# smileyenot983/reconstructor

Hardware: AMD Instinct MI355X
Metric: descriptor pair-distances/s + BA LM-iterations/s (1k cams, 100k pts) (higher is better)
Workload: dtype f16+f64

## Files before the change

reconstructor_amd/csrc/ctx.hip:

```cpp
#include "rcn_internal.h"

#include <cstdlib>

extern "C" {

const char *rcn_version(void)
{
#ifdef RCN_DIAG
    return "reconstructor_amd 0.19 (gfx950) DIAGNOSTIC BUILD";
#else
    return "reconstructor_amd 0.19 (gfx950)";
#endif
}

int rcn_create(int device_id, rcn_ctx **out)
{
    if (!out) return RCN_ERR_ARG;
    *out = nullptr;
    int n = 0;
    if (hipGetDeviceCount(&n) != hipSuccess || n <= 0 || device_id < 0 || device_id >= n)
        return RCN_ERR_NO_DEVICE;
    rcn_ctx *ctx = new rcn_ctx();
    ctx->device = device_id;
    if (hipSetDevice(device_id) != hipSuccess ||
        hipGetDeviceProperties(&ctx->prop, device_id) != hipSuccess) {
        delete ctx;
        return RCN_ERR_NO_DEVICE;
    }
    if (std::string(ctx->prop.gcnArchName).rfind("gfx950", 0) != 0) {
        delete ctx;
        return RCN_ERR_NO_DEVICE;
    }
    if (hipStreamCreateWithFlags(&ctx->own_stream, hipStreamNonBlocking) != hipSuccess) {
        delete ctx;
        return RCN_ERR_HIP;
    }
    ctx->stream = ctx->own_stream;
    if (int rcc = rcn_chol_create(ctx)) { delete ctx; return rcc; }
    if (hipEventCreateWithFlags(&ctx->ba_pair_ev, hipEventDisableTiming) != hipSuccess) { delete ctx; return RCN_ERR_HIP; }
    for (auto &e : ctx->ba_tev)
        if (hipEventCreate(&e) != hipSuccess) { delete ctx; return RCN_ERR_HIP; }
    ctx->ba_ev_made = true;
    if (hipHostMalloc(reinterpret_cast<void **>(&ctx->ba_host_scal), 16 * sizeof(double), hipHostMallocDefault) != hipSuccess) { (void)hipGetLastError(); ctx->ba_host_scal = nullptr; }
    else memset(ctx->ba_host_scal, 0, 16 * sizeof(double));
#ifdef RCN_DIAG
    const char *w4 = std::getenv("RCN_COARSE_W4");
    ctx->coarse_w4 = w4 && w4[0] == '1';
    const char *s16 = std::getenv("RCN_COARSE_S16");
    ctx->coarse_shape = s16 ? (s16[0] == '1' ? 1 : 0) : -1;
    const char *i8 = std::getenv("RCN_COARSE_I8");
    ctx->coarse_i8_off = i8 && i8[0] == '0';
    const char *i8s = std::getenv("RCN_COARSE_I8_S16");
    ctx->coarse_i8_shape = i8s ? (i8s[0] == '1' ? 1 : 0) : -1;
    const char *fe = std::getenv("RCN_FORCE_EXACT");
    ctx->force_exact = fe && fe[0] == '1';
    const char *mi8 = std::getenv("RCN_MID_I8");
    ctx->mid_i8_off = mi8 && mi8[0] == '0';
    const char *rrp = std::getenv("RCN_RERANK_PASS");
    ctx->rerank_pass = rrp && rrp[0] == '1';
    const char *flp = std::getenv("RCN_FILTER_PASS");
    ctx->filter_pass = flp && flp[0] == '1';
    const char *nio = getenv("RCN_MATCH_NO_ORDER");
    ctx->no_item_order = nio && nio[0] == '1';
    const char *ab = std::getenv("RCN_COARSE_ABL");
    ctx->ablate = ab ? std::atoi(ab) : 0;
    const char *bat = std::getenv("RCN_BA_SCHUR_ATOMICS");
    ctx->ba_atomics = bat && bat[0] == '1';
    const char *bps = getenv("RCN_PAIR_SMALL");
    if (bps) ctx->ba_pair_small = bps[0] != '0';
    const char *btf = getenv("RCN_BA_TRSV_FWD");
    ctx->ba_trsv_fwd = btf && btf[0] == '1';
    if (const char *bm = std::getenv("RCN_BA_MIRROR")) if (bm[0] == '0' && ctx->ba_host_scal) { (void)hipHostFree(ctx->ba_host_scal); ctx->ba_host_scal = nullptr; }
    const char *ch = std::getenv("RCN_CHUNK_ROWS");
    if (ch && std::atoll(ch) > 0) ctx->chunk_rows = std::atoll(ch);
    const char *mr = std::getenv("RCN_MID_ROWS");
    if (mr && std::atoll(mr) >= 0) ctx->mid_rows = std::max<long long>(1, std::atoll(mr));
#endif
    memset(&ctx->last_stats, 0, sizeof(ctx->last_stats));
    *out = ctx;
    return RCN_OK;
}

void rcn_destroy(rcn_ctx *ctx)
{
    if (!ctx) return;
    (void)hipSetDevice(ctx->device);
    (void)hipStreamSynchronize(ctx->stream);
    rcn_match_release(ctx);
    rcn_int_ham_release(ctx);
    rcn_int_guided_release(ctx);
    rcn_int_tracks_release(ctx);
    rcn_int_mvs_release(ctx);
    DevBuf *bufs[] = {&ctx->img_table, &ctx->pairs_dev, &ctx->groups_dev, &ctx->cand, &ctx->owner,
                      &ctx->fb_list, &ctx->sv_list, &ctx->counters, &ctx->out_tmp, &ctx->cnt_tmp, &ctx->scale_dev, &ctx->desc_bad, &ctx->kp_ws, &ctx->sg_ws, &ctx->sg_scores, &ctx->gnn_ws, &ctx->gnn_mdesc, &ctx->sp_ws, &ctx->sp_out, &ctx->sift_ws, &ctx->sift_pyr, &ctx->retr_ws, &ctx->retr_out, &ctx->img_ws, &ctx->orb_ws, &ctx->orb_pyr, &ctx->orb_tab};
    for (DevBuf *b : bufs) b->release();
    for (DevBuf &b : ctx->ba_ws) b.release();
    ctx->ba_loss_ws.release();
    ctx->lm_ws.release();
    ctx->tri_ws.release();
    ctx->tri_dws.release();
    ctx->fm_ws.release();
    ctx->fm_state.release();
    ctx->fm_csr.release(); ctx->fm_pairs.release();
    for (auto &kv : ctx->coords) kv.second.first.release();
    ctx->corr.release();
    ctx->corr_ws.release(); ctx->corr_hws.release(); ctx->corr_slots.release(); ctx->att_ws.release();
    if (ctx->corr_ev) (void)hipEventDestroy(ctx->corr_ev);
    ctx->lid.release(); ctx->lid_slot_off.release(); ctx->lid_hws.release(); ctx->nvt_ws.release();
    if (ctx->nvt_ev) (void)hipEventDestroy(ctx->nvt_ev);
    if (ctx->img_ev) (void)hipEventDestroy(ctx->img_ev);
// ... 50 lines not shown
```

reconstructor_amd/csrc/match.hip:

```cpp
#include "rcn_internal.h"

#include <algorithm>
#include <cmath>

typedef _Float16 half8 __attribute__((ext_vector_type(8)));
typedef float f32x16 __attribute__((ext_vector_type(16)));
typedef float f32x4 __attribute__((ext_vector_type(4)));
typedef unsigned u32x4 __attribute__((ext_vector_type(4)));

#define RCN_TBL_BYTES ((RCN_GROUP * 24 + 127) / 128 * 128)
#define RCN_NBUF 4
#define RCN_PD 2
#define RCN_CHUNK_ROWS (1ll << 27)
#define RCN_BT 64
#define RCN_PAD_HN 1.0e30f
#define RCN_I8_IDX_MASK ((1u << RCN_I8_IDX_BITS) - 1u)
#define RCN_I8_PAD_ACC ((1 << (32 - RCN_I8_IDX_BITS)) - 1)
#define RCN_I8_BT 128
#ifndef RCN_I8_EARLY_OPEN
#define RCN_I8_EARLY_OPEN 1
#endif
#define RCN_I8_RES_MAX 8.01
#define RCN_I8_M_MAX 720.0
#define RCN_I8_PEAK_MAX 8.0
// ... 1529 lines not shown
        const unsigned cnt = a.ccount[r];
        if (cnt > (unsigned)RCN_MIDCAP) {
            if (lane == 0) a.fb2_list[atomicAdd(a.fb2_count, 1u)] = e;
            continue;
        }
        const ImgDev qi = a.imgs[a.pairs[2 * pair]];
        const ImgDev ti = a.imgs[a.pairs[2 * pair + 1]];
        double b0 = INFINITY, b1 = INFINITY;
        int i0 = 0x7FFFFFFF, i1 = 0x7FFFFFFF;
        if (lane < (int)cnt) {
            i0 = a.clist[(size_t)r * RCN_MIDCAP + lane];
            b0 = exact_d2<true>(qi.f32 + (size_t)q * a.D, ti.f32 + (size_t)i0 * a.D, a.D);
            if (!(b0 < INFINITY)) { b0 = INFINITY; i0 = 0x7FFFFFFF; }
        }
        for (int o = 32; o; o >>= 1) {
            const double c0 = __shfl_xor(b0, o), c1 = __shfl_xor(b1, o);
            const int j0 = __shfl_xor(i0, o), j1 = __shfl_xor(i1, o);
            merge_top2(b0, i0, b1, i1, c0, j0, c1, j1);
        }
        if (lane == 0) a.out[(size_t)pair * a.out_stride + q] = ratio_pass(b0, b1, a.ratio) ? i0 : -1;
    }
}

__global__ void k_unique_claim(const ImgDev *__restrict__ imgs, const int32_t *__restrict__ pairs,
                               const int32_t *__restrict__ out, int64_t out_stride,
                               int32_t *__restrict__ owner, int owner_stride, int qblocks, int pair_base)
{
    const int pl = blockIdx.x / qblocks, pair = pair_base + pl;
    const int q = (blockIdx.x - pl * qblocks) * blockDim.x + threadIdx.x;
    if (q >= imgs[pairs[2 * pair]].K) return;
    const int t = out[(size_t)pair * out_stride + q];
    if (t >= 0) atomicMin(owner + (size_t)pair * owner_stride + t, q);
}

__global__ void k_unique_emit(const ImgDev *__restrict__ imgs, const int32_t *__restrict__ pairs,
                              int32_t *__restrict__ out, int64_t out_stride,
                              const int32_t *__restrict__ owner, int owner_stride,
                              int32_t *__restrict__ counts, int qblocks, int pair_base)
{
    const int pl = blockIdx.x / qblocks, pair = pair_base + pl;
    const int q = (blockIdx.x - pl * qblocks) * blockDim.x + threadIdx.x;
    if (q >= out_stride) return;
    int32_t *o = out + (size_t)pair * out_stride + q;
    bool keep = false;
    if (q < imgs[pairs[2 * pair]].K) {
        const int t = *o;
        keep = t >= 0 && owner[(size_t)pair * owner_stride + t] == q;
    }
    if (!keep) *o = -1;
    const unsigned long long m = __ballot(keep);
    if ((threadIdx.x & 63) == 0 && m) atomicAdd(counts + pair, (int)__popcll(m));
}

__global__ __launch_bounds__(256) void k_unique_pair(const ImgDev *__restrict__ imgs, const int32_t *__restrict__ pairs,
                                                     int32_t *__restrict__ out, int64_t out_stride,
                                                     int32_t *__restrict__ counts, int pair_base)
{
    __shared__ int owner[RCN_UNIQ_LDS];
    __shared__ int wsum[4];
    const int pair = pair_base + blockIdx.x, t = threadIdx.x;
    const int Kq = imgs[pairs[2 * pair]].K, Kt = imgs[pairs[2 * pair + 1]].K;
    for (int i = t; i < Kt; i += 256) owner[i] = 0x7fffffff;
    __syncthreads();
    int32_t *row = out + (size_t)pair * out_stride;
    for (int q = t; q < Kq; q += 256) {
        const int tr = row[q];
        if (tr >= 0) atomicMin(&owner[tr], q);
    }
    __syncthreads();
    int kept = 0;
    for (int q0 = 0; q0 < out_stride; q0 += 256) {
        const int q = q0 + t;
        bool keep = false;
        if (q < out_stride) {
            const int tr = q < Kq ? row[q] : -1;
            keep = tr >= 0 && owner[tr] == q;
            if (!keep && (q >= Kq || tr >= 0)) row[q] = -1;
        }
        kept += (int)__popcll(__ballot(keep));
    }
    if ((t & 63) == 0) wsum[t >> 6] = kept;
    __syncthreads();
    if (t == 0) counts[pair] = wsum[0] + wsum[1] + wsum[2] + wsum[3];
}

__global__ void k_stats_acc(unsigned *c, int mid, unsigned midrows)
{
    if (threadIdx.x != 0 || blockIdx.x != 0) return;
    c[4] += c[0];
    c[5] += c[1];
    c[6] += mid ? c[2] + (c[0] > midrows ? c[0] - midrows : 0u) : c[0];
}

static int pad_dim(int D)
{
    if (D <= 32) return 32;
    if (D <= 64) return 64;
    if (D <= 128) return 128;
    if (D <= 256) return 256;
    return 0;
}

template <typename Kernel>
static int resident_grid(rcn_ctx *ctx, Kernel kernel, int &per_cu)
{
    if (per_cu <= 0) {
        int nb = 0;
        if (hipOccupancyMaxActiveBlocksPerMultiprocessor(&nb, kernel, 64, 0) != hipSuccess || nb < 1) nb = 4;
        per_cu = nb;
    }
    return ctx->prop.multiProcessorCount * per_cu;
}
static int rerank_grid(rcn_ctx *ctx) { static int per_cu = 0; return resident_grid(ctx, k_rerank_lds, per_cu); }
static void launch_mid_exact(rcn_ctx *ctx, const MidArgs &ma, hipStream_t st)
{
    static int per_cu = 0;
    if (ma.D <= XG_ROWF) k_mid_exact<<<resident_grid(ctx, k_mid_exact, per_cu), 64, 0, st>>>(ma);
    else k_mid_exact_wide<<<ctx->prop.multiProcessorCount * 4, 256, 0, st>>>(ma);
}

static hipError_t launch_rowstats(rcn_ctx *ctx, const float *x, int rows, int D, double *nrm2, unsigned *cnt)
{
    ctx->hist_rows += rows;
    unsigned long long *mx = reinterpret_cast<unsigned long long *>(cnt + 2);
    if (D % 4 == 0 && (reinterpret_cast<uintptr_t>(x) & 15) == 0)
        k_rowstats<true><<<std::max(1, std::min((rows + 15) / 16, 4096)), 256, 0, ctx->stream>>>(x, rows, D, nrm2, cnt, mx, cnt + RCN_HIST_WORD);
    else
        k_rowstats<false><<<std::max(1, std::min((rows + 3) / 4, 4096)), 256, 0, ctx->stream>>>(x, rows, D, nrm2, cnt, mx, cnt + RCN_HIST_WORD);
    return hipGetLastError();
}

static void free_image(ImgHost &im)
{
// ... 551 lines not shown
                e = launch_coarse<128>(ctx, ca, blocks); break;
            default: e = launch_coarse<256>(ctx, ca, blocks); break;
            }
        }
    }
    RCN_HIP(e);
    if (ctx->i8_allowed) {
#ifdef RCN_DIAG
        if (ctx->coarse_i8_shape == 0) e = launch_coarse_i8<0, 0>(ctx, ca, blocks);
        else if (ctx->ablate == 1) e = launch_coarse_i8<1, 1>(ctx, ca, blocks);
        else if (ctx->ablate == 16) e = launch_coarse_i8<16, 1>(ctx, ca, blocks);
        else if (ctx->ablate == 32) e = launch_coarse_i8<32, 1>(ctx, ca, blocks);
        else
#endif
        e = launch_coarse_i8<0, 1>(ctx, ca, blocks);
        RCN_HIP(e);
    }
    return RCN_OK;
}

struct MidSource {
    const uint2 *cand;
    const unsigned long long *fb_list;
    const unsigned *fb_count;
    const float *thr_in;
    const unsigned *tacc_in;
    uint32_t midrows;
};

static int launch_mid_tier(rcn_ctx *ctx, const grid::GridPlan &pl, const RerankArgs &ra, unsigned *ccnt, const MidSource &src, bool defer_rows)
{
    const grid::MidLayout &mo = pl.mid_ws;
    const int n_slots = ctx->grid_shape.n_slots, cus = ctx->prop.multiProcessorCount;
    hipStream_t st = ctx->stream;
    char *mw = ctx->mid_ws.as<char>();
    MidArgs ma;
    memset(&ma, 0, sizeof(ma));
    ma.imgs = ra.imgs; ma.pairs = ra.pairs; ma.cand = src.cand; ma.fb_list = src.fb_list; ma.fb_count = src.fb_count;
    ma.thr_in = src.thr_in; ma.tacc_in = src.tacc_in;
    ma.sorted = (unsigned long long *)(mw + mo.sorted); ma.thr = (float *)(mw + mo.thr); ma.ccount = (unsigned *)(mw + mo.cc); ma.tacc = (unsigned *)(mw + mo.tacc);
    ma.clist = (int32_t *)(mw + mo.cl); ma.fb2_list = (unsigned long long *)(mw + mo.fb2);
    ma.hist = (unsigned *)(mw + mo.bins); ma.offs = ma.hist + (n_slots + 1); ma.cursor = ma.offs + (n_slots + 1); ma.ibase = ma.cursor + (n_slots + 1);
    ma.n_items = ccnt + 3; ma.fb2_count = ccnt + 2;
    ma.out = ra.out; ma.out_stride = ra.out_stride; ma.sc = ra.sc; ma.n_slots = n_slots; ma.kq_stride = pl.kq_stride; ma.D = ra.D;
    ma.all_to_fallback = ra.all_to_fallback; ma.idx_mask = pl.idx_mask; ma.ratio = ra.ratio; ma.midrows = src.midrows;
    if (defer_rows) {
        k_mid_defer<<<cus * 2, 256, 0, st>>>(ma, (unsigned long long *)(mw + mo.def), (float *)(mw + mo.defthr), (unsigned *)(mw + mo.deftacc), ccnt, (unsigned)mo.rows_cap);
        k_mid_defer_commit<<<1, 64, 0, st>>>(ccnt, (unsigned)mo.rows_cap);
    }
    k_mid_hist<<<cus * 4, 256, 0, st>>>(ma);
    k_mid_bins<<<1, 1024, 0, st>>>(ma);
    k_mid_scatter<<<cus * 4, 256, 0, st>>>(ma);
    k_mid_eval<<<cus * 4, 256, 0, st>>>(ma);
    if (pl.mid_i8) k_mid_eval_i8<<<dim3((unsigned)n_slots * MI8_TILES, (unsigned)pl.mid_i8_grid_y), 256, 0, st>>>(ma);
    launch_mid_exact(ctx, ma, st);
    RCN_HIP(hipGetLastError());
    k_exact_rows_lds<<<cus * 8, 64 * EX_WAVES, 0, st>>>(ra.imgs, ra.pairs, ma.fb2_list, ma.fb2_count, ra.D, ra.ratio, ra.out, ra.out_stride);
    RCN_HIP(hipGetLastError());
    return RCN_OK;
}

static int launch_unique(rcn_ctx *ctx, const grid::GridPlan &pl, const RerankArgs &ra, int32_t *counts_dev, int p0, int np)
{
    hipStream_t st = ctx->stream;
    if (pl.uniq_lds) {
        if (!pl.defer) k_unique_pair<<<np, 256, 0, st>>>(ra.imgs, ra.pairs, ra.out, ra.out_stride, counts_dev, p0);
    } else {
        const int qblocks = (pl.kq_max + 255) / 256, eblocks = (int)((ra.out_stride + 255) / 256);
        if (pl.kq_max > 0) k_unique_claim<<<dim3((unsigned)qblocks * (unsigned)np), 256, 0, st>>>(ra.imgs, ra.pairs, ra.out, ra.out_stride, ctx->owner.as<int32_t>(), pl.owner_stride, qblocks, p0);
        RCN_HIP(hipGetLastError());
        k_unique_emit<<<dim3((unsigned)eblocks * (unsigned)np), 256, 0, st>>>(ra.imgs, ra.pairs, ra.out, ra.out_stride, ctx->owner.as<int32_t>(), pl.owner_stride, counts_dev, eblocks, p0);
    }
    RCN_HIP(hipGetLastError());
    return RCN_OK;
}

int rcn_int_match_grid(rcn_ctx *ctx, const int32_t *pairs_host, int32_t n_pairs, float ratio,
                           int32_t *out_dev, int64_t out_stride, int32_t *counts_dev)
{
    if (!pairs_host && n_pairs > 0) {
        std::vector<int32_t> ids;
        for (const auto &kv : ctx->images)
            if (kv.first != INT32_MIN && kv.first != INT32_MIN + 1) ids.push_back(kv.first);
        const int64_t want = (int64_t)ids.size() * ((int64_t)ids.size() - 1) / 2;
        if (want != n_pairs) { ctx->set_error("rcn_match_grid: pairs == NULL needs n_pairs = n (n - 1) / 2 over the resident images"); return RCN_ERR_ARG; }
        std::vector<int32_t> &all = ctx->all_pairs_host;
        all.clear();
        for (size_t i = 0; i < ids.size(); ++i)
            for (size_t j = i + 1; j < ids.size(); ++j) { all.push_back(ids[i]); all.push_back(ids[j]); }
        pairs_host = all.data();
    }
    if (n_pairs < 0 || (n_pairs > 0 && (!pairs_host || !out_dev || !counts_dev))) {
        ctx->set_error("rcn_match_grid: bad argument");
        return RCN_ERR_ARG;
    }
    memset(&ctx->last_stats, 0, sizeof(ctx->last_stats));
    if (n_pairs == 0) return RCN_OK;
    RCN_HIP(hipSetDevice(ctx->device));
    int rc = rcn_int_prepare_all(ctx);
    if (rc) return rc;

    if ((rc = fill_grid_shape(ctx, pairs_host, n_pairs))) return rc;
    const grid::GridShape &gs = ctx->grid_shape;
    grid::GridPlan &pl = ctx->grid;
    grid::plan_grid(gs, pl);
    if (out_stride < pl.kq_max) {
        ctx->set_error("rcn_match_grid: out_stride smaller than a query image's K");
// ... 365 lines not shown
{
    if (!ctx || !model) return RCN_ERR_ARG;
    std::lock_guard<std::mutex> lk(ctx->mu);
    if (!ctx->scale_dev.p || !ctx->prepared) { ctx->set_error("rcn_diag_i8: nothing prepared"); return RCN_ERR_ARG; }
    RCN_HIP(hipSetDevice(ctx->device));
    ScaleDev m;
    RCN_HIP(hipMemcpyAsync(&m, ctx->scale_dev.p, sizeof(ScaleDev), hipMemcpyDeviceToHost, ctx->stream));
    RCN_HIP(hipStreamSynchronize(ctx->stream));
    model[0] = m.coarse_i8; model[1] = m.s; model[2] = m.bias; model[3] = m.rho; model[4] = m.tau; model[5] = m.n_max;
    model[6] = ctx->i8_allowed ? 1.0 : 0.0; model[7] = 0.0;
    if (!q_host && !hn_host && !norms_host) return RCN_OK;
    auto it = ctx->images.find(img_id);
    if (it == ctx->images.end()) { ctx->set_error("rcn_diag_i8: image id not resident"); return RCN_ERR_NOT_FOUND; }
    if (!m.coarse_i8 || !it->second.i8n) { ctx->set_error("rcn_diag_i8: the resident set holds no int8 copies"); return RCN_ERR_UNSUPPORTED; }
    const ImgHost &im = it->second;
    if (im.K <= 0) return RCN_OK;
    std::vector<int8_t> raw((size_t)im.K * 256);
    std::vector<float> nn((size_t)im.K * 2);
    RCN_HIP(hipMemcpyAsync(raw.data(), im.f16, raw.size(), hipMemcpyDeviceToHost, ctx->stream));
    if (hn_host) RCN_HIP(hipMemcpyAsync(hn_host, im.hn, (size_t)im.K * sizeof(int32_t), hipMemcpyDeviceToHost, ctx->stream));
    RCN_HIP(hipMemcpyAsync(nn.data(), im.i8n, nn.size() * sizeof(float), hipMemcpyDeviceToHost, ctx->stream));
    RCN_HIP(hipStreamSynchronize(ctx->stream));
    if (q_host)
        for (int r = 0; r < im.K; ++r)
            for (int c = 0; c < 16; ++c) memcpy(q_host + (size_t)r * 256 + 16 * c, raw.data() + (size_t)r * 256 + ((c ^ (r & 15)) << 4), 16);
    if (norms_host) memcpy(norms_host, nn.data(), nn.size() * sizeof(float));
    return RCN_OK;
}
#endif

#ifdef RCN_DIAG
int rcn_diag_mid(rcn_ctx *ctx, int64_t *n_rows, unsigned long long *sorted_host, uint32_t *tacc_host, uint32_t *ccount_host, int32_t *clist_host, int64_t cap)
{
    if (!ctx || !n_rows) return RCN_ERR_ARG;
    std::lock_guard<std::mutex> lk(ctx->mu);
    if (!ctx->grid.mid || !ctx->mid_ws.p || ctx->last_chunks != 1) { ctx->set_error("rcn_diag_mid: the last grid call left no single pass of the middle tier"); return RCN_ERR_UNSUPPORTED; }
    RCN_HIP(hipSetDevice(ctx->device));
    const grid::MidLayout &mo = ctx->grid.mid_ws;
    unsigned c0 = 0;
    RCN_HIP(hipMemcpyAsync(&c0, ctx->counters.as<unsigned>() + 8, sizeof(unsigned), hipMemcpyDeviceToHost, ctx->stream));
    RCN_HIP(hipStreamSynchronize(ctx->stream));
    const size_t n = std::min<size_t>(c0, mo.rows_cap);
    *n_rows = (int64_t)n;
    if (n == 0 || (!sorted_host && !tacc_host && !ccount_host && !clist_host)) return RCN_OK;
    if ((int64_t)n > cap) { ctx->set_error("rcn_diag_mid: the arrays are too short"); return RCN_ERR_ARG; }
    const char *mw = ctx->mid_ws.as<char>();
    if (sorted_host) RCN_HIP(hipMemcpyAsync(sorted_host, mw + mo.sorted, n * 8, hipMemcpyDeviceToHost, ctx->stream));
    if (tacc_host) RCN_HIP(hipMemcpyAsync(tacc_host, mw + mo.tacc, n * 4, hipMemcpyDeviceToHost, ctx->stream));
    if (ccount_host) RCN_HIP(hipMemcpyAsync(ccount_host, mw + mo.cc, n * 4, hipMemcpyDeviceToHost, ctx->stream));
    if (clist_host) RCN_HIP(hipMemcpyAsync(clist_host, mw + mo.cl, n * 4 * RCN_MIDCAP, hipMemcpyDeviceToHost, ctx->stream));
    RCN_HIP(hipStreamSynchronize(ctx->stream));
    return RCN_OK;
}
#endif

int rcn_match_set_workspace_rows(rcn_ctx *ctx, int64_t rows)
{
    if (!ctx || rows < 0) return RCN_ERR_ARG;
    std::lock_guard<std::mutex> lk(ctx->mu);
    ctx->chunk_rows = rows == 0 ? RCN_CHUNK_ROWS : std::max<int64_t>(rows, 1);
    return RCN_OK;
}

int rcn_match_profile(rcn_ctx *ctx, int enable)
{
    if (!ctx) return RCN_ERR_ARG;
    std::lock_guard<std::mutex> lk(ctx->mu);
    RCN_HIP(hipSetDevice(ctx->device));
    if (enable && !ctx->ev_made) {
        for (auto &call : ctx->ev_c)
            for (auto &row : call)
                for (auto &e : row) RCN_HIP(hipEventCreate(&e));
        for (auto &row : ctx->ev_tail)
            for (auto &e : row) RCN_HIP(hipEventCreate(&e));
        ctx->ev_made = true;
    }
    ctx->profile = enable != 0;
    ctx->ev_n = 0;
    return RCN_OK;
}

}
```

reconstructor_amd/csrc/mid_i8.h:

```cpp
#pragma once

#define MI8_QB 32

__global__ __launch_bounds__(256, 2) void k_mid_eval_i8(MidArgs a)
{
    __shared__ uint4 qs[2][MI8_QB * 16];
    __shared__ int qthr[2][MI8_QB];
    if (!a.sc->coarse_i8) return;
    const int t = threadIdx.x;
    const int bin = blockIdx.x / MI8_TILES, tile = blockIdx.x - bin * MI8_TILES;
    const unsigned first = a.offs[bin], h = a.offs[bin + 1] - first;
    const int nb = (int)((h + MI8_QB - 1) / MI8_QB);
    if ((int)blockIdx.y >= nb) return;
    const ImgDev ti = a.imgs[bin];
    if (tile * MI8_TR >= ti.Kp) return;

    unsigned tr[2][64];
    int hn[2], jrow[2];
#pragma unroll
    for (int k = 0; k < 2; ++k) {
        const int j = tile * MI8_TR + k * 256 + t;
        jrow[k] = j;
        const bool in = j < ti.Kp;
        hn[k] = in ? reinterpret_cast<const int *>(ti.hn)[j] : RCN_I8_PAD_ACC;
        const char *row = reinterpret_cast<const char *>(ti.f16) + (size_t)(in ? j : 0) * 256;
#pragma unroll
        for (int c = 0; c < 16; ++c) {
            uint4 v = make_uint4(0u, 0u, 0u, 0u);
            if (in) v = *reinterpret_cast<const uint4 *>(row + ((c ^ (j & 15)) << 4));
            tr[k][4 * c] = v.x; tr[k][4 * c + 1] = v.y; tr[k][4 * c + 2] = v.z; tr[k][4 * c + 3] = v.w;
        }
    }

    const int qr = t >> 3, c0 = (t & 7) * 2;
    uint4 f0, f1;
    int fthr;
    auto fetch = [&](int b) {
        const unsigned i = (unsigned)b * MI8_QB + (unsigned)qr;
        f0 = make_uint4(0u, 0u, 0u, 0u); f1 = f0; fthr = -1;
        if (i < h) {
            const unsigned ta = a.tacc[first + i];
            if (ta) {
                const unsigned long long e = a.sorted[first + i];
                const int pair = (int)(e >> 32), q = (int)(e & 0xFFFFFFFFu);
                const char *row = reinterpret_cast<const char *>(a.imgs[a.pairs[2 * pair]].f16) + (size_t)q * 256;
                f0 = *reinterpret_cast<const uint4 *>(row + ((c0 ^ (q & 15)) << 4));
                f1 = *reinterpret_cast<const uint4 *>(row + (((c0 + 1) ^ (q & 15)) << 4));
                fthr = (int)ta;
            }
        }
    };
    auto stage = [&](int buf) {
        qs[buf][qr * 16 + c0] = f0;
        qs[buf][qr * 16 + c0 + 1] = f1;
        if ((t & 7) == 0) qthr[buf][qr] = fthr;
    };
    int b = (int)blockIdx.y, buf = 0;
    fetch(b);
    stage(0);
    __syncthreads();
    for (; b < nb; b += (int)gridDim.y, buf ^= 1) {
        const bool more = b + (int)gridDim.y < nb;
        if (more) fetch(b + (int)gridDim.y);
        for (int r = 0; r < MI8_QB; ++r) {
            const int thr = __builtin_amdgcn_readfirstlane(qthr[buf][r]);
            if (thr < 0) continue;
            int d0 = 0, d1 = 0;
#pragma unroll
            for (int c = 0; c < 16; ++c) {
                const uint4 x = qs[buf][r * 16 + c];
                d0 = __builtin_amdgcn_sdot4((int)x.x, (int)tr[0][4 * c], d0, false);
                d1 = __builtin_amdgcn_sdot4((int)x.x, (int)tr[1][4 * c], d1, false);
                d0 = __builtin_amdgcn_sdot4((int)x.y, (int)tr[0][4 * c + 1], d0, false);
                d1 = __builtin_amdgcn_sdot4((int)x.y, (int)tr[1][4 * c + 1], d1, false);
                d0 = __builtin_amdgcn_sdot4((int)x.z, (int)tr[0][4 * c + 2], d0, false);
                d1 = __builtin_amdgcn_sdot4((int)x.z, (int)tr[1][4 * c + 2], d1, false);
                d0 = __builtin_amdgcn_sdot4((int)x.w, (int)tr[0][4 * c + 3], d0, false);
                d1 = __builtin_amdgcn_sdot4((int)x.w, (int)tr[1][4 * c + 3], d1, false);
            }
            const unsigned slot = first + (unsigned)b * MI8_QB + (unsigned)r;
#pragma unroll
            for (int k = 0; k < 2; ++k) {
                const int acc = hn[k] - (k ? d1 : d0);
                if (acc <= thr && jrow[k] < ti.K) {
                    const unsigned pos = atomicAdd(a.ccount + slot, 1u);
                    if (pos < (unsigned)RCN_MIDCAP) a.clist[(size_t)slot * RCN_MIDCAP + pos] = jrow[k];
                }
            }
        }
        if (more) stage(buf ^ 1);
        __syncthreads();
    }
}
```

reconstructor_amd/csrc/rcn_internal.h:

```cpp
#pragma once
#include <hip/hip_runtime.h>
#include <hip/hip_fp16.h>
#include <array>
#include <cstdint>
#include <cstdio>
#include <cstring>
#include <map>
#include <mutex>
#include <string>
#include <vector>

#include "../../include/rcn.h"
#include "grid_plan.h"

#define RCN_HIP(call)                                                                    \
    do {                                                                                 \
        hipError_t e_ = (call);                                                          \
        if (e_ != hipSuccess) {                                                          \
            ctx->set_error(std::string(#call) + ": " + hipGetErrorString(e_));           \
            return RCN_ERR_HIP;                                                          \
        }                                                                                \
    } while (0)

struct DevBuf {
// ... 138 lines not shown
    DevBuf sg_ws, sg_scores;
    int64_t sg_chunk_bytes = 0;
    DevBuf gnn_ws, gnn_mdesc;
    int32_t gnn_chunk_pairs = 0;
    DevBuf sp_ws, sp_out;
    int32_t sp_chunk_images = 0;
    DevBuf sift_ws, sift_pyr;
    int32_t sift_chunk_images = 0;
    DevBuf orb_ws, orb_pyr, orb_tab;
    int32_t orb_chunk_images = 0;
    std::vector<int64_t> orb_tab_key;
    DevBuf retr_ws, retr_out;
    DevBuf img_ws;
    std::vector<char> img_stage_host;
    hipEvent_t img_ev = nullptr;
    bool img_stage_pending = false;
    ScaleDev scale_host;
    bool scale_on_device = false;
    bool want_dev_scale = false;
    bool i8_allowed = false;
    int32_t coarse_i8_host = 0;
    std::vector<ImgDev> table_host;
    DevBuf img_table, pairs_dev, groups_dev, cand, owner, fb_list, sv_list, counters, out_tmp, cnt_tmp;
    hipEvent_t f32_ready = nullptr;
    DevBuf cmp_off, cmp_qt[2];
    hipStream_t copy_stream = nullptr;
    hipEvent_t cmp_ev[2] = {nullptr, nullptr}, cmp_filled = nullptr;
    bool cmp_busy[2] = {false, false};
    int cmp_next = 0, cmp_last = -1;
    int32_t last_kq_stride = 0, last_n_pairs = 0;
    uint32_t last_idx_mask = 0;
    rcn_match_stats last_stats;
    bool profile = false;
#define RCN_EV_CHUNKS 64
    hipEvent_t ev_c[64][RCN_EV_CHUNKS][4];
    hipEvent_t ev_tail[64][3];
    bool ev_tail_on[64] = {false};
    int ev_chunks[64] = {0};
    int last_chunks = 1;
    int64_t chunk_rows = 1ll << 27;
    int64_t mid_rows = 1ll << 21;
    DevBuf mid_ws;
    int mid_bins_slots = -1;
    bool ev_made = false;
    int ev_n = 0;
#ifdef RCN_DIAG
    bool coarse_w4 = false;
    bool coarse_i8_off = false;
    int coarse_i8_shape = -1;
    int coarse_shape = -1;
    int ablate = 0;
    bool force_exact = false;
    bool mid_i8_off = false;
    bool rerank_pass = false;
    bool filter_pass = false;
    bool no_item_order = false;
    bool ba_atomics = false;
    bool ba_trsv_fwd = false;
    bool ba_pair_small = true;
#else
    static constexpr bool coarse_w4 = false;
    static constexpr bool coarse_i8_off = false;
    static constexpr int coarse_i8_shape = -1;
    static constexpr int coarse_shape = -1;
    static constexpr int ablate = 0;
    static constexpr bool mid_i8_off = false, rerank_pass = false, filter_pass = false;
    static constexpr bool force_exact = false, no_item_order = false, ba_atomics = false, ba_trsv_fwd = false, ba_pair_small = true;
#endif

    DevBuf ba_ws[40];
    DevBuf ba_loss_ws;
    DevBuf lm_ws;
    DevBuf tri_ws, tri_dws;
    DevBuf fm_ws, fm_state;
    std::vector<PairXY> fm_pairs_host;
    DevBuf fm_csr, fm_pairs;
    DevBuf gd_pairs, gd_ws, gd_hws, gd_F;
    std::vector<char> gd_pairs_host;
    std::map<int32_t, std::pair<DevBuf, int32_t>> coords;
    CorrLists corr;
    DevBuf corr_ws, corr_hws, corr_slots, att_ws;
    std::vector<char> corr_slots_host;
    hipEvent_t corr_ev = nullptr;
    bool corr_slots_pending = false;
    DevBuf pnp_hws, pnp_slots;
    std::vector<char> pnp_slots_host;
    hipEvent_t pnp_ev = nullptr;
    bool pnp_slots_pending = false;
    DevBuf tv_hws, tv_dws, tv_fws;
    DevBuf hg_hws, hg_dws;
    std::vector<char> tv_stage_host;
    hipEvent_t tv_ev = nullptr;
    bool tv_stage_pending = false;
    int64_t corr_budget = 1ll << 30;
    DevBuf lid, lid_slot_off, lid_hws;
    std::map<int32_t, std::pair<int64_t, int32_t>> lid_rows;
    bool lid_live = false;
    uint64_t coords_gen = 0, lists_gen = 0;
    uint64_t lid_coords_gen = 0, lid_lists_gen = 0;
    DevBuf nvt_ws;
    std::vector<char> nvt_stage_host;
    hipEvent_t nvt_ev = nullptr;
    bool nvt_stage_pending = false;
    std::vector<int> ba_graph_cam, ba_graph_pt;
    int ba_graph_nc = 0, ba_graph_np = 0;
    uint64_t ba_graph_serial = 0;
// ... 120 lines not shown
```

reconstructor_amd/csrc/store.hip:

```cpp
#include "rcn_internal.h"
#include "wgprim.h"

#include <cerrno>
#include <cstdio>
#include <cstdlib>

namespace {

__global__ __launch_bounds__(1024) void k_cmp_scan(const int32_t *__restrict__ counts, int n, long long *__restrict__ off)
{
    const long long total = wg_scan_array(counts, n, off, 0ll);
    if (threadIdx.x == 1023) off[n] = total;
}

__global__ __launch_bounds__(256) void k_cmp_fill(const int32_t *__restrict__ table, int64_t stride,
                                                  const int32_t *__restrict__ counts, const long long *__restrict__ off,
                                                  int2 *__restrict__ qt)
{
    __shared__ int wsum[4];
    const int pair = blockIdx.x, t = threadIdx.x;
    const int total = counts[pair];
    if (total <= 0) return;
    const int32_t *row = table + (size_t)pair * stride;
    int2 *dst = qt + off[pair];
    int pos = 0;
    for (int64_t q0 = 0; q0 < stride && pos < total; q0 += 256) {
        const int64_t q = q0 + t;
        const int tr = q < stride ? row[q] : -1;
        int chunk;
        const int at = pos + wg_rank<256>(tr >= 0, wsum, chunk);
        if (tr >= 0 && at < total) dst[at] = make_int2((int)q, tr);
        pos += chunk;
    }
}

}

extern "C" {

int rcn_host_alloc(void **out, size_t bytes)
{
    if (!out) return RCN_ERR_ARG;
    *out = nullptr;
    if (hipHostMalloc(out, bytes ? bytes : 1, hipHostMallocDefault) != hipSuccess) { (void)hipGetLastError(); return RCN_ERR_HIP; }
    return RCN_OK;
}

void rcn_host_free(void *p)
{
    if (p) (void)hipHostFree(p);
}

int rcn_match_compact_begin(rcn_ctx *ctx, const int32_t *table_dev, int64_t stride, const int32_t *counts_dev,
                            int32_t n_pairs, int64_t *offsets_host, int32_t *qt_host, int64_t capacity, int64_t *total_out)
{
    if (!ctx) return RCN_ERR_ARG;
    std::lock_guard<std::mutex> lk(ctx->mu);
    return rcn_int_compact_begin(ctx, table_dev, stride, counts_dev, n_pairs, offsets_host, qt_host, capacity, total_out);
}

int rcn_match_compact_wait(rcn_ctx *ctx)
{
    if (!ctx) return RCN_ERR_ARG;
    std::lock_guard<std::mutex> lk(ctx->mu);
    return rcn_int_compact_wait(ctx);
}

}

void rcn_int_launch_cmp_fill(hipStream_t st, const int32_t *table_dev, int64_t stride, const int32_t *counts_dev, const long long *off, int32_t n_pairs, int2 *qt)
{
    k_cmp_fill<<<n_pairs, 256, 0, st>>>(table_dev, stride, counts_dev, off, qt);
}

int rcn_int_compact_begin(rcn_ctx *ctx, const int32_t *table_dev, int64_t stride, const int32_t *counts_dev,
                          int32_t n_pairs, int64_t *offsets_host, int32_t *qt_host, int64_t capacity, int64_t *total_out)
{
    if (n_pairs < 0 || stride < 0 || capacity < 0 || !offsets_host || !total_out ||
        (n_pairs > 0 && (!table_dev || !counts_dev)) || (capacity > 0 && !qt_host)) {
        ctx->set_error("rcn_match_compact_begin: bad argument");
        return RCN_ERR_ARG;
    }
    *total_out = 0;
    offsets_host[0] = 0;
    if (n_pairs == 0) return RCN_OK;
    RCN_HIP(hipSetDevice(ctx->device));
    if (!ctx->copy_stream) {
        RCN_HIP(hipStreamCreateWithFlags(&ctx->copy_stream, hipStreamNonBlocking));
        for (auto &e : ctx->cmp_ev) RCN_HIP(hipEventCreateWithFlags(&e, hipEventDisableTiming));
        RCN_HIP(hipEventCreateWithFlags(&ctx->cmp_filled, hipEventDisableTiming));
    }
    hipStream_t st = ctx->stream;
    RCN_HIP(ctx->cmp_off.reserve(sizeof(long long) * ((size_t)n_pairs + 1)));
    long long *off = ctx->cmp_off.as<long long>();
    k_cmp_scan<<<1, 1024, 0, st>>>(counts_dev, n_pairs, off);
    RCN_HIP(hipGetLastError());
    static_assert(sizeof(long long) == sizeof(int64_t), "offset type");
    RCN_HIP(hipMemcpyAsync(offsets_host, off, sizeof(int64_t) * ((size_t)n_pairs + 1), hipMemcpyDeviceToHost, st));
    RCN_HIP(hipStreamSynchronize(st));
    const int64_t total = offsets_host[n_pairs];
    *total_out = total;
    if (total > capacity) {
        ctx->set_error("rcn_match_compact_begin: qt_host holds fewer entries than the table has matches");
        return RCN_ERR_ARG;
    }
    if (total == 0) return RCN_OK;
    const int b = 0;
    if (ctx->cmp_busy[b]) RCN_HIP(hipStreamWaitEvent(st, ctx->cmp_ev[b], 0));
    if ((size_t)total * sizeof(int2) > ctx->cmp_qt[b].cap) {
        if (ctx->cmp_busy[b]) RCN_HIP(hipEventSynchronize(ctx->cmp_ev[b]));
        RCN_HIP(ctx->cmp_qt[b].reserve((size_t)total * sizeof(int2)));
    }
    k_cmp_fill<<<n_pairs, 256, 0, st>>>(table_dev, stride, counts_dev, off, ctx->cmp_qt[b].as<int2>());
    RCN_HIP(hipGetLastError());
    RCN_HIP(hipEventRecord(ctx->cmp_filled, st));
    RCN_HIP(hipStreamWaitEvent(ctx->copy_stream, ctx->cmp_filled, 0));
    RCN_HIP(hipMemcpyAsync(qt_host, ctx->cmp_qt[b].p, (size_t)total * sizeof(int2), hipMemcpyDeviceToHost, ctx->copy_stream));
    RCN_HIP(hipEventRecord(ctx->cmp_ev[b], ctx->copy_stream));
    ctx->cmp_busy[b] = true;
    ctx->cmp_last = b;
    return RCN_OK;
}

int rcn_int_compact_wait(rcn_ctx *ctx)
{
    if (ctx->cmp_last >= 0 && ctx->cmp_busy[ctx->cmp_last]) RCN_HIP(hipEventSynchronize(ctx->cmp_ev[ctx->cmp_last]));
    return RCN_OK;
}

extern "C" {

struct StoreHeader {
    char magic[8];
    uint32_t version, endian;
    int32_t n_images, D, has_coords, n_pairs;
    int64_t total_matches;
    char zero[24];
};
static_assert(sizeof(StoreHeader) == 64, "store header is 64 bytes");

}

struct rcn_store {
    std::vector<char> bytes;
    StoreHeader h;
    std::vector<int32_t> ids, Ks;
    std::vector<const float *> desc;
    std::vector<const int32_t *> coords;
    const int32_t *pairs = nullptr;
    const int64_t *offsets = nullptr;
    const int32_t *qt = nullptr;
};

namespace {

struct Fnv {
    uint64_t h = 1469598103934665603ull;
    void add(const void *p, size_t n)
    {
        const unsigned char *b = static_cast<const unsigned char *>(p);
        for (size_t i = 0; i < n; ++i) { h ^= b[i]; h *= 1099511628211ull; }
    }
};

struct Writer {
    FILE *f;
// ... 148 lines not shown
```

Before: 5376 billion.

## Use i8 MFMA for mid-stage eval, vectorize unique-pair and compaction fill

Replaces the default mid-stage int8 distance kernel with one that computes query-vs-tile dot products using 16x16x64 i8 MFMA instructions, with a swizzled LDS layout and negated query bytes so that each accumulator, seeded with the row term, can be compared directly against the threshold. The old dot4 kernel stays available only behind a diagnostic env flag. Separately, k_unique_pair and k_cmp_fill now read four ints per thread with int4 loads, keep small rows in registers, and count survivors with a wave shuffle reduction. The aim is to raise int8 throughput and cut scalar memory traffic, in exchange for more register pressure and new layout code that has to be correct.

```diff
diff --git a/reconstructor_amd/csrc/ctx.hip b/reconstructor_amd/csrc/ctx.hip
--- a/reconstructor_amd/csrc/ctx.hip
+++ b/reconstructor_amd/csrc/ctx.hip
@@ -56,6 +56,8 @@
     ctx->force_exact = fe && fe[0] == '1';
     const char *mi8 = std::getenv("RCN_MID_I8");
     ctx->mid_i8_off = mi8 && mi8[0] == '0';
+    const char *mi8m = std::getenv("RCN_MID_I8_MFMA");
+    ctx->mid_i8_dot4 = mi8m && mi8m[0] == '0';
     const char *rrp = std::getenv("RCN_RERANK_PASS");
     ctx->rerank_pass = rrp && rrp[0] == '1';
     const char *flp = std::getenv("RCN_FILTER_PASS");
diff --git a/reconstructor_amd/csrc/match.hip b/reconstructor_amd/csrc/match.hip
--- a/reconstructor_amd/csrc/match.hip
+++ b/reconstructor_amd/csrc/match.hip
@@ -1605,33 +1605,72 @@
     if ((threadIdx.x & 63) == 0 && m) atomicAdd(counts + pair, (int)__popcll(m));
 }
 
+#define UQ_REG_ROWS 4096
+static_assert(RCN_UNIQ_LDS % 4 == 0 && UQ_REG_ROWS % 1024 == 0, "the owner table and a register row are whole groups");
+__device__ __forceinline__ void uq_claim4(const int4 v, int q0, int Kq, int *owner)
+{
+    if (q0 < Kq && v.x >= 0) atomicMin(&owner[v.x], q0);
+    if (q0 + 1 < Kq && v.y >= 0) atomicMin(&owner[v.y], q0 + 1);
+    if (q0 + 2 < Kq && v.z >= 0) atomicMin(&owner[v.z], q0 + 2);
+    if (q0 + 3 < Kq && v.w >= 0) atomicMin(&owner[v.w], q0 + 3);
+}
+__device__ __forceinline__ int uq_emit4(int32_t *at, const int4 v, int q0, int Kq, const int *owner)
+{
+    auto stay = [&](int tr, int q) { return q < Kq ? (tr < 0 || owner[tr] == q ? tr : -1) : -1; };
+    const int4 n = make_int4(stay(v.x, q0), stay(v.y, q0 + 1), stay(v.z, q0 + 2), stay(v.w, q0 + 3));
+    if (n.x != v.x || n.y != v.y || n.z != v.z || n.w != v.w) *reinterpret_cast<int4 *>(at) = n;
+    return (n.x >= 0) + (n.y >= 0) + (n.z >= 0) + (n.w >= 0);
+}
 __global__ __launch_bounds__(256) void k_unique_pair(const ImgDev *__restrict__ imgs, const int32_t *__restrict__ pairs,
                                                      int32_t *__restrict__ out, int64_t out_stride,
                                                      int32_t *__restrict__ counts, int pair_base)
 {
-    __shared__ int owner[RCN_UNIQ_LDS];
+    __shared__ __attribute__((aligned(16))) int owner[RCN_UNIQ_LDS];
     __shared__ int wsum[4];
     const int pair = pair_base + blockIdx.x, t = threadIdx.x;
     const int Kq = imgs[pairs[2 * pair]].K, Kt = imgs[pairs[2 * pair + 1]].K;
-    for (int i = t; i < Kt; i += 256) owner[i] = 0x7fffffff;
+    const int4 nobody = make_int4(0x7fffffff, 0x7fffffff, 0x7fffffff, 0x7fffffff);
+    for (int i = t; 4 * i < Kt; i += 256) reinterpret_cast<int4 *>(owner)[i] = nobody;
     __syncthreads();
     int32_t *row = out + (size_t)pair * out_stride;
-    for (int q = t; q < Kq; q += 256) {
-        const int tr = row[q];
-        if (tr >= 0) atomicMin(&owner[tr], q);
-    }
-    __syncthreads();
     int kept = 0;
-    for (int q0 = 0; q0 < out_stride; q0 += 256) {
-        const int q = q0 + t;
-        bool keep = false;
-        if (q < out_stride) {
+    if ((out_stride & 3) == 0 && (reinterpret_cast<uintptr_t>(out) & 15) == 0) {
+        if (out_stride <= UQ_REG_ROWS) {
+            int4 v[UQ_REG_ROWS / 1024];
+#pragma unroll
+            for (int k = 0; k < UQ_REG_ROWS / 1024; ++k) {
+                const int q0 = 4 * (k * 256 + t);
+                v[k] = make_int4(-1, -1, -1, -1);
+                if (q0 < out_stride) v[k] = *reinterpret_cast<const int4 *>(row + q0);
+            }
+#pragma unroll
+            for (int k = 0; k < UQ_REG_ROWS / 1024; ++k) uq_claim4(v[k], 4 * (k * 256 + t), Kq, owner);
+            __syncthreads();
+#pragma unroll
+            for (int k = 0; k < UQ_REG_ROWS / 1024; ++k) {
+                const int q0 = 4 * (k * 256 + t);
+                if (q0 < out_stride) kept += uq_emit4(row + q0, v[k], q0, Kq, owner);
+            }
+        } else {
+            for (int q0 = 4 * t; q0 < Kq; q0 += 1024) uq_claim4(*reinterpret_cast<const int4 *>(row + q0), q0, Kq, owner);
+            __syncthreads();
+            for (int q0 = 4 * t; q0 < out_stride; q0 += 1024) kept += uq_emit4(row + q0, *reinterpret_cast<const int4 *>(row + q0), q0, Kq, owner);
+        }
+    } else {
+        for (int q = t; q < Kq; q += 256) {
+            const int tr = row[q];
+            if (tr >= 0) atomicMin(&owner[tr], q);
+        }
+        __syncthreads();
+        for (int q = t; q < out_stride; q += 256) {
             const int tr = q < Kq ? row[q] : -1;
-            keep = tr >= 0 && owner[tr] == q;
+            const bool keep = tr >= 0 && owner[tr] == q;
             if (!keep && (q >= Kq || tr >= 0)) row[q] = -1;
-        }
-        kept += (int)__popcll(__ballot(keep));
-    }
+            kept += keep;
+        }
+    }
+#pragma unroll
+    for (int o = 32; o; o >>= 1) kept += __shfl_xor(kept, o);
     if ((t & 63) == 0) wsum[t >> 6] = kept;
     __syncthreads();
     if (t == 0) counts[pair] = wsum[0] + wsum[1] + wsum[2] + wsum[3];
@@ -2289,7 +2328,15 @@
     k_mid_bins<<<1, 1024, 0, st>>>(ma);
     k_mid_scatter<<<cus * 4, 256, 0, st>>>(ma);
     k_mid_eval<<<cus * 4, 256, 0, st>>>(ma);
-    if (pl.mid_i8) k_mid_eval_i8<<<dim3((unsigned)n_slots * MI8_TILES, (unsigned)pl.mid_i8_grid_y), 256, 0, st>>>(ma);
+    if (pl.mid_i8) {
+        const dim3 g8((unsigned)n_slots * MI8_TILES, (unsigned)pl.mid_i8_grid_y);
+#ifdef RCN_DIAG
+        ctx->mid_i8_launched = ctx->mid_i8_dot4 ? 2 : 1;
+        if (ctx->mid_i8_dot4) k_mid_eval_i8_dot4<<<g8, 256, 0, st>>>(ma);
+        else
+#endif
+        k_mid_eval_i8<<<g8, 256, 0, st>>>(ma);
+    }
     launch_mid_exact(ctx, ma, st);
     RCN_HIP(hipGetLastError());
     k_exact_rows_lds<<<cus * 8, 64 * EX_WAVES, 0, st>>>(ra.imgs, ra.pairs, ma.fb2_list, ma.fb2_count, ra.D, ra.ratio, ra.out, ra.out_stride);
@@ -2761,6 +2808,45 @@
     RCN_HIP(hipStreamSynchronize(ctx->stream));
     return RCN_OK;
 }
+
+int rcn_diag_mid_sweep(rcn_ctx *ctx)
+{
+    if (!ctx) return RCN_ERR_ARG;
+    std::lock_guard<std::mutex> lk(ctx->mu);
+    return ctx->mid_i8_launched;
+}
+
+int rcn_diag_unique_pair(rcn_ctx *ctx, const int32_t *kq_kt_host, int32_t n_pairs, int32_t *table_dev, int64_t stride, int32_t *counts_dev)
+{
+    if (!ctx || n_pairs < 0 || (n_pairs > 0 && (!kq_kt_host || !table_dev || !counts_dev))) return RCN_ERR_ARG;
+    if (n_pairs == 0) return RCN_OK;
+    std::lock_guard<std::mutex> lk(ctx->mu);
+    std::vector<ImgDev> imgs(2 * (size_t)n_pairs);
+    std::vector<int32_t> pr(2 * (size_t)n_pairs);
+    for (int i = 0; i < 2 * n_pairs; ++i) {
+        const int32_t k = kq_kt_host[i];
+        if (k < 0 || ((i & 1) ? k > RCN_UNIQ_LDS : k > stride)) { ctx->set_error("rcn_diag_unique_pair: a row count the kernel does not take"); return RCN_ERR_ARG; }
+        memset(&imgs[i], 0, sizeof(ImgDev));
+        imgs[i].K = k;
+        pr[i] = i;
+    }
+    RCN_HIP(hipSetDevice(ctx->device));
+    ImgDev *di = nullptr;
+    int32_t *dp = nullptr;
+    if (hipMalloc(&di, imgs.size() * sizeof(ImgDev)) != hipSuccess || hipMalloc(&dp, pr.size() * sizeof(int32_t)) != hipSuccess) { (void)hipFree(di); return RCN_ERR_HIP; }
+    hipError_t e = hipMemcpyAsync(di, imgs.data(), imgs.size() * sizeof(ImgDev), hipMemcpyHostToDevice, ctx->stream);
+    if (e == hipSuccess) e = hipMemcpyAsync(dp, pr.data(), pr.size() * sizeof(int32_t), hipMemcpyHostToDevice, ctx->stream);
+    if (e == hipSuccess) {
+        k_unique_pair<<<n_pairs, 256, 0, ctx->stream>>>(di, dp, table_dev, stride, counts_dev, 0);
+        e = hipGetLastError();
+    }
+    const hipError_t es = hipStreamSynchronize(ctx->stream);
+    (void)hipFree(di);
+    (void)hipFree(dp);
+    RCN_HIP(e);
+    RCN_HIP(es);
+    return RCN_OK;
+}
 #endif
 
 int rcn_match_set_workspace_rows(rcn_ctx *ctx, int64_t rows)
diff --git a/reconstructor_amd/csrc/mid_i8.h b/reconstructor_amd/csrc/mid_i8.h
--- a/reconstructor_amd/csrc/mid_i8.h
+++ b/reconstructor_amd/csrc/mid_i8.h
@@ -1,8 +1,133 @@
 #pragma once
+#include "mid_i8_addr.h"
 
 #define MI8_QB 32
+static_assert(MI8_QB == (int)mi8addr::BATCH_ROWS && MI8_TR == (int)mi8addr::TILE_ROWS && RCN_QT % MI8_TR == 0, "mid_i8_addr.h describes this tile");
+
+template <bool NEG, bool SWZ> struct Mi8Batch {
+    uint4 f0, f1;
+    int fthr;
+    __device__ __forceinline__ void fetch(const MidArgs &a, unsigned first, unsigned h, int b)
+    {
+        const int t = threadIdx.x, qr = t >> 3, c0 = (t & 7) * 2;
+        const unsigned i = (unsigned)b * MI8_QB + (unsigned)qr;
+        f0 = make_uint4(0u, 0u, 0u, 0u); f1 = f0; fthr = -1;
+        if (i < h) {
+            const unsigned ta = a.tacc[first + i];
+            if (ta) {
+                const unsigned long long e = a.sorted[first + i];
+                const int pair = (int)(e >> 32), q = (int)(e & 0xFFFFFFFFu);
+                const char *row = reinterpret_cast<const char *>(a.imgs[a.pairs[2 * pair]].f16) + (size_t)q * 256;
+                f0 = *reinterpret_cast<const uint4 *>(row + ((c0 ^ (q & 15)) << 4));
+                f1 = *reinterpret_cast<const uint4 *>(row + (((c0 + 1) ^ (q & 15)) << 4));
+                if (NEG) {
+                    f0.x = neg_i8x4(f0.x); f0.y = neg_i8x4(f0.y); f0.z = neg_i8x4(f0.z); f0.w = neg_i8x4(f0.w);
+                    f1.x = neg_i8x4(f1.x); f1.y = neg_i8x4(f1.y); f1.z = neg_i8x4(f1.z); f1.w = neg_i8x4(f1.w);
+                }
+                fthr = (int)ta;
+            }
+        }
+    }
+    __device__ __forceinline__ void stage(uint4 *qs, int *qthr) const
+    {
+        const int t = threadIdx.x, qr = t >> 3, c0 = (t & 7) * 2;
+        if (SWZ) {
+            qs[mi8addr::q_off((unsigned)qr, (unsigned)c0) >> 4] = f0;
+            qs[mi8addr::q_off((unsigned)qr, (unsigned)c0 + 1u) >> 4] = f1;
+        } else {
+            qs[qr * 16 + c0] = f0;
+            qs[qr * 16 + c0 + 1] = f1;
+        }
+        if ((t & 7) == 0) qthr[qr] = fthr;
+    }
+};
 
 __global__ __launch_bounds__(256, 2) void k_mid_eval_i8(MidArgs a)
+{
+    __shared__ uint4 qs[2][MI8_QB * 16];
+    __shared__ int qthr[2][MI8_QB];
+    if (!a.sc->coarse_i8) return;
+    const int t = threadIdx.x, lane = t & 63, w = t >> 6, r = lane & 15, h4 = lane >> 4;
+    const int bin = blockIdx.x / MI8_TILES, tile = blockIdx.x - bin * MI8_TILES;
+    const unsigned first = a.offs[bin], h = a.offs[bin + 1] - first;
+    const int nb = (int)((h + MI8_QB - 1) / MI8_QB);
+    if ((int)blockIdx.y >= nb) return;
+    const ImgDev ti = a.imgs[bin];
+    if (tile * MI8_TR >= ti.Kp) return;
+
+    i32x4 av[8][4], hnv[8];
+    {
+        const char *tb = reinterpret_cast<const char *>(ti.f16) + (size_t)tile * MI8_TR * 256;
+        const int *hb = reinterpret_cast<const int *>(ti.hn) + tile * MI8_TR;
+#pragma unroll
+        for (int rb = 0; rb < 8; ++rb) {
+#pragma unroll
+            for (int ks = 0; ks < 4; ++ks)
+                av[rb][ks] = *reinterpret_cast<const i32x4 *>(tb + mi8addr::a_off((unsigned)w, (unsigned)rb, (unsigned)r, (unsigned)h4, (unsigned)ks));
+            const int *hp = hb + mi8addr::tile_row((unsigned)w, (unsigned)rb, 4u * (unsigned)h4);
+            hnv[rb] = i32x4{hp[0], hp[1], hp[2], hp[3]};
+        }
+    }
+    const int row0 = tile * MI8_TR + (int)mi8addr::tile_row((unsigned)w, 0u, 4u * (unsigned)h4);
+
+    Mi8Batch<true, true> f;
+    int b = (int)blockIdx.y, buf = 0;
+    f.fetch(a, first, h, b);
+    f.stage(qs[0], qthr[0]);
+    __syncthreads();
+    for (; b < nb; b += (int)gridDim.y, buf ^= 1) {
+        const bool more = b + (int)gridDim.y < nb;
+        if (more) f.fetch(a, first, h, b + (int)gridDim.y);
+        int thr[2];
+#pragma unroll
+        for (int cb = 0; cb < 2; ++cb) {
+            const int v = qthr[buf][16 * cb + r];
+            thr[cb] = v < 0 ? (int)0x80000000 : v;
+        }
+        if (__ballot(thr[0] != (int)0x80000000 || thr[1] != (int)0x80000000)) {
+            i32x4 bq[2][4];
+            const char *qb = reinterpret_cast<const char *>(qs[buf]);
+#pragma unroll
+            for (int cb = 0; cb < 2; ++cb)
+#pragma unroll
+                for (int ks = 0; ks < 4; ++ks)
+                    bq[cb][ks] = *reinterpret_cast<const i32x4 *>(qb + mi8addr::b_off((unsigned)cb, (unsigned)r, (unsigned)h4, (unsigned)ks));
+            const unsigned slot0 = first + (unsigned)b * MI8_QB + (unsigned)r;
+#pragma unroll
+            for (int rp = 0; rp < 4; ++rp) {
+                i32x4 c[2][2];
+#pragma unroll
+                for (int ks = 0; ks < 4; ++ks)
+#pragma unroll
+                    for (int i = 0; i < 2; ++i)
+#pragma unroll
+                        for (int cb = 0; cb < 2; ++cb)
+                            c[i][cb] = __builtin_amdgcn_mfma_i32_16x16x64_i8(av[2 * rp + i][ks], bq[cb][ks], ks == 0 ? hnv[2 * rp + i] : c[i][cb], 0, 0, 0);
+#pragma unroll
+                for (int i = 0; i < 2; ++i)
+#pragma unroll
+                    for (int cb = 0; cb < 2; ++cb) {
+                        const i32x4 v = c[i][cb];
+                        if (min(min(v[0], v[1]), min(v[2], v[3])) > thr[cb]) continue;
+#pragma unroll
+                        for (int reg = 0; reg < 4; ++reg) {
+                            const int j = row0 + 16 * (2 * rp + i) + reg;
+                            if (v[reg] <= thr[cb] && j < ti.K) {
+                                const unsigned slot = slot0 + 16u * (unsigned)cb;
+                                const unsigned pos = atomicAdd(a.ccount + slot, 1u);
+                                if (pos < (unsigned)RCN_MIDCAP) a.clist[(size_t)slot * RCN_MIDCAP + pos] = j;
+                            }
+                        }
+                    }
+            }
+        }
+        if (more) f.stage(qs[buf ^ 1], qthr[buf ^ 1]);
+        __syncthreads();
+    }
+}
+
+#ifdef RCN_DIAG
+__global__ __launch_bounds__(256, 2) void k_mid_eval_i8_dot4(MidArgs a)
 {
     __shared__ uint4 qs[2][MI8_QB * 16];
     __shared__ int qthr[2][MI8_QB];
@@ -32,36 +157,14 @@
         }
     }
 
-    const int qr = t >> 3, c0 = (t & 7) * 2;
-    uint4 f0, f1;
-    int fthr;
-    auto fetch = [&](int b) {
-        const unsigned i = (unsigned)b * MI8_QB + (unsigned)qr;
-        f0 = make_uint4(0u, 0u, 0u, 0u); f1 = f0; fthr = -1;
-        if (i < h) {
-            const unsigned ta = a.tacc[first + i];
-            if (ta) {
-                const unsigned long long e = a.sorted[first + i];
-                const int pair = (int)(e >> 32), q = (int)(e & 0xFFFFFFFFu);
-                const char *row = reinterpret_cast<const char *>(a.imgs[a.pairs[2 * pair]].f16) + (size_t)q * 256;
-                f0 = *reinterpret_cast<const uint4 *>(row + ((c0 ^ (q & 15)) << 4));
-                f1 = *reinterpret_cast<const uint4 *>(row + (((c0 + 1) ^ (q & 15)) << 4));
-                fthr = (int)ta;
-            }
-        }
-    };
-    auto stage = [&](int buf) {
-        qs[buf][qr * 16 + c0] = f0;
-        qs[buf][qr * 16 + c0 + 1] = f1;
-        if ((t & 7) == 0) qthr[buf][qr] = fthr;
-    };
+    Mi8Batch<false, false> f;
     int b = (int)blockIdx.y, buf = 0;
-    fetch(b);
-    stage(0);
+    f.fetch(a, first, h, b);
+    f.stage(qs[0], qthr[0]);
     __syncthreads();
     for (; b < nb; b += (int)gridDim.y, buf ^= 1) {
         const bool more = b + (int)gridDim.y < nb;
-        if (more) fetch(b + (int)gridDim.y);
+        if (more) f.fetch(a, first, h, b + (int)gridDim.y);
         for (int r = 0; r < MI8_QB; ++r) {
             const int thr = __builtin_amdgcn_readfirstlane(qthr[buf][r]);
             if (thr < 0) continue;
@@ -88,7 +191,8 @@
                 }
             }
         }
-        if (more) stage(buf ^ 1);
+        if (more) f.stage(qs[buf ^ 1], qthr[buf ^ 1]);
         __syncthreads();
     }
 }
+#endif
diff --git a/reconstructor_amd/csrc/mid_i8_addr.h b/reconstructor_amd/csrc/mid_i8_addr.h
--- /dev/null
+++ b/reconstructor_amd/csrc/mid_i8_addr.h
@@ -0,0 +1,30 @@
+#pragma once
+
+#if defined(__HIPCC__) || defined(__CUDACC__)
+#define RCN_MI8A_FN __host__ __device__ constexpr
+#else
+#define RCN_MI8A_FN constexpr
+#endif
+
+namespace mi8addr {
+
+constexpr unsigned ROW_BYTES = 256;
+constexpr unsigned TILE_ROWS = 512;
+constexpr unsigned WAVES = 4;
+constexpr unsigned WAVE_ROWS = TILE_ROWS / WAVES;
+constexpr unsigned ROW_BLOCKS = WAVE_ROWS / 16;
+constexpr unsigned BATCH_ROWS = 32;
+constexpr unsigned COL_BLOCKS = BATCH_ROWS / 16;
+constexpr unsigned K_STEPS = ROW_BYTES / 64;
+
+RCN_MI8A_FN unsigned tile_row(unsigned w, unsigned rb, unsigned i) { return w * WAVE_ROWS + rb * 16u + i; }
+RCN_MI8A_FN unsigned chunk_off(unsigned row, unsigned c) { return ((c ^ (row & 15u)) << 4); }
+RCN_MI8A_FN unsigned frag_chunk(unsigned h, unsigned ks) { return 4u * ks + h; }
+RCN_MI8A_FN unsigned a_off(unsigned w, unsigned rb, unsigned r, unsigned h, unsigned ks) { return tile_row(w, rb, r) * ROW_BYTES + chunk_off(tile_row(w, rb, r), frag_chunk(h, ks)); }
+RCN_MI8A_FN unsigned q_off(unsigned s, unsigned c) { return s * ROW_BYTES + chunk_off(s, c); }
+RCN_MI8A_FN unsigned b_off(unsigned cb, unsigned r, unsigned h, unsigned ks) { return q_off(16u * cb + r, frag_chunk(h, ks)); }
+
+static_assert(TILE_ROWS % (16 * WAVES) == 0 && BATCH_ROWS % 16 == 0, "whole 16-row blocks");
+static_assert(b_off(COL_BLOCKS - 1, 15, 3, K_STEPS - 1) < BATCH_ROWS * ROW_BYTES, "a B fragment stays inside its buffer");
+
+}
diff --git a/reconstructor_amd/csrc/rcn_internal.h b/reconstructor_amd/csrc/rcn_internal.h
--- a/reconstructor_amd/csrc/rcn_internal.h
+++ b/reconstructor_amd/csrc/rcn_internal.h
@@ -214,6 +214,8 @@
     int ablate = 0;
     bool force_exact = false;
     bool mid_i8_off = false;
+    bool mid_i8_dot4 = false;
+    int mid_i8_launched = 0;
     bool rerank_pass = false;
     bool filter_pass = false;
     bool no_item_order = false;
diff --git a/reconstructor_amd/csrc/store.hip b/reconstructor_amd/csrc/store.hip
--- a/reconstructor_amd/csrc/store.hip
+++ b/reconstructor_amd/csrc/store.hip
@@ -13,6 +13,7 @@
     if (threadIdx.x == 1023) off[n] = total;
 }
 
+template <bool VEC>
 __global__ __launch_bounds__(256) void k_cmp_fill(const int32_t *__restrict__ table, int64_t stride,
                                                   const int32_t *__restrict__ counts, const long long *__restrict__ off,
                                                   int2 *__restrict__ qt)
@@ -24,14 +25,38 @@
     const int32_t *row = table + (size_t)pair * stride;
     int2 *dst = qt + off[pair];
     int pos = 0;
-    for (int64_t q0 = 0; q0 < stride && pos < total; q0 += 256) {
-        const int64_t q = q0 + t;
-        const int tr = q < stride ? row[q] : -1;
-        int chunk;
-        const int at = pos + wg_rank<256>(tr >= 0, wsum, chunk);
-        if (tr >= 0 && at < total) dst[at] = make_int2((int)q, tr);
-        pos += chunk;
-    }
+    if (VEC) {
+        const int4 none = make_int4(-1, -1, -1, -1);
+        int4 v = 4 * t < stride ? *reinterpret_cast<const int4 *>(row + 4 * t) : none;
+        for (int64_t q0 = 0; q0 < stride && pos < total; q0 += 1024) {
+            const int64_t q = q0 + 4 * t, qn = q + 1024;
+            const int4 nx = qn < stride ? *reinterpret_cast<const int4 *>(row + qn) : none;
+            const int mine = (v.x >= 0) + (v.y >= 0) + (v.z >= 0) + (v.w >= 0);
+            int chunk;
+            int at = pos + wg_scan_incl<int, 256>(mine, wsum, chunk) - mine;
+            if (v.x >= 0) { if (at < total) dst[at] = make_int2((int)q, v.x); ++at; }
+            if (v.y >= 0) { if (at < total) dst[at] = make_int2((int)q + 1, v.y); ++at; }
+            if (v.z >= 0) { if (at < total) dst[at] = make_int2((int)q + 2, v.z); ++at; }
+            if (v.w >= 0 && at < total) dst[at] = make_int2((int)q + 3, v.w);
+            pos += chunk;
+            v = nx;
+        }
+    } else {
+        for (int64_t q0 = 0; q0 < stride && pos < total; q0 += 256) {
+            const int64_t q = q0 + t;
+            const int tr = q < stride ? row[q] : -1;
+            int chunk;
+            const int at = pos + wg_rank<256>(tr >= 0, wsum, chunk);
+            if (tr >= 0 && at < total) dst[at] = make_int2((int)q, tr);
+            pos += chunk;
+        }
+    }
+}
+
+void launch_cmp_fill(hipStream_t st, const int32_t *table, int64_t stride, const int32_t *counts, const long long *off, int32_t n_pairs, int2 *qt)
+{
+    if ((stride & 3) == 0 && (reinterpret_cast<uintptr_t>(table) & 15) == 0) k_cmp_fill<true><<<n_pairs, 256, 0, st>>>(table, stride, counts, off, qt);
+    else k_cmp_fill<false><<<n_pairs, 256, 0, st>>>(table, stride, counts, off, qt);
 }
 
 }
@@ -70,7 +95,7 @@
 
 void rcn_int_launch_cmp_fill(hipStream_t st, const int32_t *table_dev, int64_t stride, const int32_t *counts_dev, const long long *off, int32_t n_pairs, int2 *qt)
 {
-    k_cmp_fill<<<n_pairs, 256, 0, st>>>(table_dev, stride, counts_dev, off, qt);
+    launch_cmp_fill(st, table_dev, stride, counts_dev, off, n_pairs, qt);
 }
 
 int rcn_int_compact_begin(rcn_ctx *ctx, const int32_t *table_dev, int64_t stride, const int32_t *counts_dev,
@@ -111,7 +136,7 @@
         if (ctx->cmp_busy[b]) RCN_HIP(hipEventSynchronize(ctx->cmp_ev[b]));
         RCN_HIP(ctx->cmp_qt[b].reserve((size_t)total * sizeof(int2)));
     }
-    k_cmp_fill<<<n_pairs, 256, 0, st>>>(table_dev, stride, counts_dev, off, ctx->cmp_qt[b].as<int2>());
+    launch_cmp_fill(st, table_dev, stride, counts_dev, off, n_pairs, ctx->cmp_qt[b].as<int2>());
     RCN_HIP(hipGetLastError());
     RCN_HIP(hipEventRecord(ctx->cmp_filled, st));
     RCN_HIP(hipStreamWaitEvent(ctx->copy_stream, ctx->cmp_filled, 0));
```

Result: faster. 5453 billion (median of 6 runs) (+1.4%).
